# peterropac/Aegolius

Hardware: AMD Instinct MI355X
Metric: Mpoints/sec SDF eval, 1024^3 grid, 10-prim smooth-union tree (higher is better)
Workload: dtype f32

## Files before the change

### aegolius_amd/_engine.py

```python
import atexit
import contextlib
import ctypes
import importlib.util
import os
import sys
import threading

import numpy as np

_HERE = os.path.dirname(os.path.abspath(__file__))
LIB_PATH = os.path.join(_HERE, "libsdfk.so")

MODE_AUTO, MODE_INTERPRET, MODE_SPECIALIZED, MODE_NOCULL = 0, 1, 2, 3
(FLAVOUR_PLAIN_ARRAY, FLAVOUR_PLAIN_GRID, FLAVOUR_TILE_ARRAY, FLAVOUR_TILE_GRID, FLAVOUR_TILE_MASK, FLAVOUR_ROWS_ARRAY,
 FLAVOUR_ROWS_GRID, FLAVOUR_ROWS_MASK, FLAVOUR_ROWS2D_ARRAY, FLAVOUR_ROWS2D_GRID, FLAVOUR_RAYS, FLAVOUR_OCCUPANCY) = range(12)
FLAVOUR_FLAGS = 0x100
FLAVOUR_XY = 0x200

_c = ctypes
_vp, _i64, _int, _sz = _c.c_void_p, _c.c_int64, _c.c_int, _c.c_size_t
_fp = _c.POINTER(_c.c_float)

SIGNATURES = {
    "sdfk_abi_version": (_int, []),
    "sdfk_device_count": (_int, []),
    "sdfk_last_error": (_c.c_char_p, []),
    "sdfk_program_create": (_vp, [_vp, _sz, _vp, _sz, _vp, _sz, _int]),
    "sdfk_program_destroy": (None, [_vp]),
    "sdfk_program_set_params": (_int, [_vp, _vp, _sz]),
    "sdfk_program_set_cull": (_int, [_vp, _vp, _sz, _vp]),
    "sdfk_program_source": (_c.c_char_p, [_vp]),
    "sdfk_program_compile_check": (_int, [_vp, _c.POINTER(_sz)]),
    "sdfk_program_chain_members": (_int, [_vp]),
    "sdfk_program_compile_flavour": (_int, [_vp, _int, _c.POINTER(_sz), _c.POINTER(_c.c_double)]),
    "sdfk_debug_compile_external": (_int, [_vp, _int, _c.POINTER(_sz)]),
    "sdfk_debug_jit_stats": (None, [_c.POINTER(_i64), _c.POINTER(_c.c_double)]),
    "sdfk_jit_drain": (None, []),
    "sdfk_jit_cancel": (None, []),
    "sdfk_debug_set_rtc_defs": (None, [_c.c_char_p]),
    "sdfk_eval_device": (_int, [_vp, _vp, _i64, _i64, _vp, _vp, _int]),
    "sdfk_eval_device_rows": (_int, [_vp, _vp, _i64, _i64, _i64, _vp, _vp, _int]),
    "sdfk_eval_device_rows2d": (_int, [_vp, _vp, _i64, _i64, _i64, _vp, _vp, _int]),
    "sdfk_eval_device_rows2d_xy": (_int, [_vp, _vp, _i64, _i64, _i64, _vp, _vp, _int]),
    "sdfk_debug_cells_stats": (None, [_int, _c.POINTER(_c.c_longlong)]),
    "sdfk_debug_rays_stats": (None, [_int, _c.POINTER(_c.c_longlong)]),
    "sdfk_eval_device_rows3d": (_int, [_vp, _vp, _i64, _i64, _i64, _i64, _i64, _vp, _vp, _int]),
    "sdfk_debug_row_masks": (_int, [_vp, _vp, _i64, _i64, _i64, _vp, _c.POINTER(_i64), _c.POINTER(_int), _vp]),
    "sdfk_eval_grid_sharded": (_int, [_vp, _vp, _i64, _vp, _i64, _vp, _i64, _int, _vp, _vp, _int]),
    "sdfk_eval_grid_sharded_device": (_int, [_vp, _vp, _i64, _vp, _i64, _vp, _i64, _int, _vp, _int, _vp, _int]),
    "sdfk_eval_device_aux": (_int, [_vp, _vp, _i64, _i64, _vp, _int, _i64, _vp, _vp, _int]),
    "sdfk_eval_grid_aux": (_int, [_vp, _vp, _i64, _vp, _i64, _vp, _i64, _i64, _i64, _vp, _int, _i64, _vp, _vp, _int]),
    "sdfk_field_min": (_int, [_vp, _i64, _c.POINTER(_c.c_float), _vp]),
    "sdfk_grid_box_average": (_int, [_vp, _i64, _i64, _i64, _int, _int, _int, _int, _vp, _vp]),
    "sdfk_grid_edge_detect": (_int, [_vp, _i64, _i64, _i64, _vp, _vp]),
    "sdfk_debug_box_variant": (_int, [_i64, _i64, _i64, _int, _int, _int, _c.POINTER(_int)]),
    "sdfk_grid_signed": (_int, [_vp, _i64, _i64, _i64, _c.c_float, _int, _vp, _vp]),
    "sdfk_grid_boundary_mask": (_int, [_vp, _i64, _c.c_float, _vp, _vp]),
    "sdfk_grid_signed_slab": (_int, [_vp, _i64, _i64, _vp, _i64, _i64, _i64, _int, _vp, _vp]),
    "sdfk_eval_host": (_int, [_vp, _vp, _int, _i64, _i64, _vp, _int, _int]),
# ... 720 lines not shown
```

### aegolius_amd/csrc/sdfk.hip

```cpp
#include <hip/hip_runtime.h>
#include <hip/hiprtc.h>

#include <chrono>
#include <algorithm>
#include <atomic>
#include <cmath>
#include <condition_variable>
#include <cstdio>
#include <cstdlib>
#include <cstring>
#include <deque>
#include <functional>
#include <map>
#include <memory>
#include <mutex>
#include <thread>
#include <string>
#include <vector>
#include <dirent.h>
#include <dlfcn.h>
#include <fcntl.h>
#include <signal.h>
#include <spawn.h>
#include <sys/wait.h>
// ... 1045 lines not shown
    }
    e->cv.notify_all();
}
template <typename MakeSource>
static std::shared_ptr<CodeObject> code_get(const std::string& key, MakeSource make_source, int rwb, bool wait) {
    std::shared_ptr<CodeObject> e = code_entry(key);
    std::unique_lock<std::mutex> lk(e->mu);
    if (e->state == 3 && std::chrono::steady_clock::now() - e->failed_at > std::chrono::seconds(30)) e->state = 0;
    if (e->state == 0) {
        e->state = 1;
        lk.unlock();
        const std::string src = make_source();
        if (wait || !rtc_helper_available()) {
            code_build(e, src, rwb);
        } else {
            g_builds.post([e, src, rwb] { code_build(e, src, rwb, true); });
        }
        return e;
    }
    if (wait) e->cv.wait(lk, [&] { return e->state != 1; });
    return e;
}
static std::string flavour_key(const sdfk_program* p, int flavour, int rwb, int with_flags = 0) {
    return p->key + "|f" + std::to_string(flavour) + ((with_flags & 1) ? "s" : "") + ((with_flags & 2) ? "x" : "") + "|" + rtc_option_key(rwb);
}
static std::string flavour_source(const sdfk_program* p, int flavour, int with_flags = 0) {
    return std::string((with_flags & 1) ? "#define SDFK_FLAGS 1\n" : "") + ((with_flags & 2) ? "#define SDFK_XY 1\n" : "") +
           sdfk_generate_source(g_ops, SDFK_OP_COUNT, p->code.data(), p->code.size() / 2, p->result_reg, p->sites, flavour,
                                &p->sites_all);
}

extern "C" int sdfk_program_chain_members(const sdfk_program* p) {
    return p && p->chain_mode ? p->chain_members : 0;
}
extern "C" int sdfk_program_compile_check(sdfk_program* p, size_t* code_size) {
    if (!p) return fail(-1, "null program");
    size_t total = 0;
    const int rwb = rows_geo(p);
    for (int f = 0; f < SDFK_FL_COUNT; ++f) {
        if (f == SDFK_FL_RAYS) continue;
        if (f == SDFK_FL_OCCUPANCY) continue;
        if (p->sites.empty() && f != SDFK_FL_PLAIN_ARRAY && f != SDFK_FL_PLAIN_GRID) continue;
        if (p->chain_mode && (f == SDFK_FL_TILE_ARRAY || f == SDFK_FL_TILE_GRID || f == SDFK_FL_TILE_MASK || f == SDFK_FL_ROWS_MASK)) continue;
        std::shared_ptr<CodeObject> e = code_get(flavour_key(p, f, rwb), [&] { return flavour_source(p, f); }, rwb, true);
        if (e->state != 2) return fail(-3, e->error);
        total += e->co.size();
    }
    if (code_size) *code_size = total;
    return 0;
}
extern "C" int sdfk_program_compile_flavour(sdfk_program* p, int flavour, size_t* code_size, double* seconds) {
    if (!p) return fail(-1, "null program");
    int with_flags = 0;
    if (flavour >= 0 && (flavour & SDFK_FLAVOUR_FLAGS)) with_flags |= 1;
    if (flavour >= 0 && (flavour & SDFK_FLAVOUR_XY)) with_flags |= 2;
    if (flavour >= 0) flavour &= ~(SDFK_FLAVOUR_FLAGS | SDFK_FLAVOUR_XY);
    if (flavour < 0 || flavour >= SDFK_FL_COUNT) return fail(-1, "sdfk_program_compile_flavour: unknown flavour");
    if (p->sites.empty() && flavour != SDFK_FL_PLAIN_ARRAY && flavour != SDFK_FL_PLAIN_GRID && flavour != SDFK_FL_RAYS &&
        flavour != SDFK_FL_OCCUPANCY)
        return fail(-2, "sdfk_program_compile_flavour: the program has no cull sites");
    if (with_flags && flavour == SDFK_FL_RAYS)
        return fail(-2, "sdfk_program_compile_flavour: the ray flavour has no flag-writing or two-row build");
    if (with_flags && flavour == SDFK_FL_OCCUPANCY)
        return fail(-2, "sdfk_program_compile_flavour: the occupancy flavour has no flag-writing or two-row build");
    if ((with_flags & 2) && flavour != SDFK_FL_PLAIN_ARRAY && flavour != SDFK_FL_ROWS2D_ARRAY)
        return fail(-2, "sdfk_program_compile_flavour: two-row coordinates exist for the plain and the flat row-block array kernels");
    if ((with_flags & 1) && (flavour == SDFK_FL_TILE_ARRAY || flavour == SDFK_FL_TILE_GRID || flavour == SDFK_FL_TILE_MASK ||
                       flavour == SDFK_FL_ROWS_MASK))
        return fail(-2, "sdfk_program_compile_flavour: this flavour has no flag-writing build");
    const int rwb = rows_geo(p);
    const auto t0 = std::chrono::steady_clock::now();
    std::shared_ptr<CodeObject> e =
        code_get(flavour_key(p, flavour, rwb, with_flags), [&] { return flavour_source(p, flavour, with_flags); }, rwb, true);
    if (e->state != 2) return fail(-3, e->error);
    if (code_size) *code_size = e->co.size();
    if (seconds) *seconds = std::chrono::duration<double>(std::chrono::steady_clock::now() - t0).count();
    return 0;
}

extern "C" int sdfk_debug_compile_external(sdfk_program* p, int flavour, size_t* code_size) {
    if (!p) return fail(-1, "null program");
    if (flavour < 0 || flavour >= SDFK_FL_COUNT) return fail(-1, "sdfk_debug_compile_external: unknown flavour");
    if (p->sites.empty() && flavour != SDFK_FL_PLAIN_ARRAY && flavour != SDFK_FL_PLAIN_GRID && flavour != SDFK_FL_RAYS &&
        flavour != SDFK_FL_OCCUPANCY)
        return fail(-2, "sdfk_debug_compile_external: the program has no cull sites");
    if (!rtc_helper_available()) return fail(-9, "sdfk_rtc_helper is not next to libsdfk.so (or hiprtc cannot be located)");
    std::vector<char> co;
    std::string log;
    if (rtc_compile_external(flavour_source(p, flavour), &co, &log, rows_geo(p)) != 0) return fail(-3, log);
    if (code_size) *code_size = co.size();
    return 0;
}

static std::shared_ptr<SpecModule> get_module(sdfk_program* p, int device, int flavour, bool wait, std::string* err,
                                              int with_flags = 0) {
    const int rwb = rows_geo(p);
    const std::string key = flavour_key(p, flavour, rwb, with_flags);
    std::shared_ptr<SpecModule> m;
    {
        std::lock_guard<std::mutex> lk(g_code_mu);
        std::shared_ptr<SpecModule>& slot = g_mods[std::make_pair(device, key)];
        if (!slot) slot = std::make_shared<SpecModule>();
        m = slot;
    }
    std::lock_guard<std::mutex> lk(m->mu);
    if (m->loaded) return m;
    for (int attempt = 0;; ++attempt) {
        std::shared_ptr<CodeObject> e;
        {
            std::lock_guard<std::mutex> ce(g_code_mu);
            auto it = g_code.find(key);
            if (it != g_code.end()) e = it->second;
// ... 232 lines not shown
        for (const uint2& x : sp) {
            if (x.y == 0xffffffffu) ++all;
            else { sum += x.y; mx = std::max<unsigned long long>(mx, x.y); if (x.y == 0) ++empty; }
        }
        {
            std::lock_guard<std::mutex> lk(g_cells_stats_mu);
            g_cells_stats[0] = (long long)nf; g_cells_stats[1] = (long long)nc; g_cells_stats[2] = (long long)head;
            g_cells_stats[3] = (long long)cap; g_cells_stats[4] = (long long)sum; g_cells_stats[5] = (long long)mx;
            g_cells_stats[6] = (long long)all; g_cells_stats[7] = (long long)empty;
        }
        if (trace) fprintf(stderr, "[sdfk cells] %d members: fine %ux%ux%u = %llu cells (2^%u planes x 2^%u blocks x 2^%u windows), coarse %llu; pool %u of %llu entries; "
                "fine lists: mean %.1f max %llu, %llu without a list, %llu empty\n", p->chain_members, fine.ncx, fine.ncy, fine.ncz, nf, fine.lx, fine.ly, fine.lz, nc,
                head, cap, (double)sum / (double)std::max<unsigned long long>(1, nf - all - empty), mx, all, empty);
    }
    out->lv = fine;
    out->sph = b + o_fsph;
    out->span = b + o_fspan;
    out->cand = b + o_pool;
    out->enabled = 1u;
    out->ncells = (unsigned)nf;
    return 0;
}

static int run(sdfk_program* p, const SrcArray* arr, const SrcGrid* grid, long long n, float* d_out, void* stream_,
               int mode, bool vec_ok, long long row_len = 0, const float* aux = nullptr, long long aux_stride = 0,
               bool flat = false, long long plane_rows = 0, long long plane_phase = 0, unsigned* d_flags = nullptr,
               unsigned thr_key = 0, bool xy = false) {
    if (!p) return fail(-1, "null program");
    if (n < 0) return fail(-1, "negative point count");
    if (p->n_aux > 0 && (!aux || aux_stride < n))
        return fail(-1, "this program reads auxiliary fields (staged evaluation): use sdfk_eval_device_aux / sdfk_eval_grid_aux");
    if (n == 0) return 0;
    if (mode == SDFK_MODE_AUTO) mode = g_default_mode;
    if (d_flags && (mode == SDFK_MODE_AUTO || mode == SDFK_MODE_INTERPRET)) mode = SDFK_MODE_SPECIALIZED;
    if (xy) {
        if (!arr || p->n_aux > 0) return fail(-1, "two-row coordinates: array source, no auxiliary fields");
        if (mode == SDFK_MODE_AUTO || mode == SDFK_MODE_INTERPRET) mode = SDFK_MODE_SPECIALIZED;
    }
    hipStream_t stream = (hipStream_t)stream_;
    int device = 0;
    HIPCHK(hipGetDevice(&device));
    DevState* d = nullptr;
    int rc = ensure_resident(p, device, stream, &d);
    if (rc) return rc;

    long long n4 = vec_ok ? (n / 4) * 4 : 0;
    long long tail = n - n4;

    static const long long spec_limit = [] {
        const char* e = getenv("SDFK_SPECIALIZE_LIMIT");
// ... 12 lines not shown
    int flavour = arr ? SDFK_FL_PLAIN_ARRAY : SDFK_FL_PLAIN_GRID;
    const long long grow = grid ? (grid->n2 > 1 ? (long long)grid->n2 : (long long)grid->n1) : 0;
    if (!p->sites.empty() && mode != SDFK_MODE_NOCULL && mode != SDFK_MODE_INTERPRET) {
        if (arr && rows_geometry(n, row_len, &rg, (flat || d_flags) ? 0 : plane_rows, plane_phase, p->chain_mode))
            flavour = (flat || xy) ? SDFK_FL_ROWS2D_ARRAY : SDFK_FL_ROWS_ARRAY;
        else if (arr && vec_ok && !p->chain_mode && !d_flags && !xy) flavour = SDFK_FL_TILE_ARRAY;
        else if (grid && grid->start % grow == 0 &&
                 rows_geometry(n, grow, &rg, (grid->n2 > 1 && !d_flags) ? (long long)grid->n1 : 0,
                               grid->n2 > 1 ? (grid->start / grow) % (long long)grid->n1 : 0, p->chain_mode))
            flavour = grid->n2 > 1 ? SDFK_FL_ROWS_GRID : SDFK_FL_ROWS2D_GRID;
        else if (grid && vec_ok && !p->chain_mode && !d_flags) flavour = SDFK_FL_TILE_GRID;
        if (!p->chain_mode && (long long)(p->code.size() / 2) > rows_limit &&
            (flavour == SDFK_FL_ROWS_ARRAY || flavour == SDFK_FL_ROWS2D_ARRAY || flavour == SDFK_FL_ROWS_GRID || flavour == SDFK_FL_ROWS2D_GRID)) {
            const bool is_arr = arr != nullptr;
            if (vec_ok && !d_flags && !xy) flavour = is_arr ? SDFK_FL_TILE_ARRAY : SDFK_FL_TILE_GRID;
            else if (!d_flags) flavour = is_arr ? SDFK_FL_PLAIN_ARRAY : SDFK_FL_PLAIN_GRID;
        }
    }
    std::shared_ptr<SpecModule> sk;
    if (mode != SDFK_MODE_INTERPRET) {
        static const bool async_jit = [] { const char* e = getenv("SDFK_ASYNC_JIT"); return !(e && e[0] == '0'); }();
        const bool wait = mode != SDFK_MODE_AUTO || !p->interp_ok || !async_jit;
        std::string err;
        sk = get_module(p, device, flavour, wait, &err, (d_flags ? 1 : 0) | (xy ? 2 : 0));
        if (sk && sk->failed) {
            if (mode == SDFK_MODE_SPECIALIZED || !p->interp_ok)
                return fail(-3, "specialised kernel unavailable: " + err);
            static bool warned = false;
            if (!warned) {
                fprintf(stderr, "[sdfk] hiprtc specialisation failed, using the interpreter kernel: %s\n", err.c_str());
                warned = true;
            }
            sk.reset();
        }
    }
    if (!sk && !p->interp_ok)
        return fail(-4, "program needs more registers than the interpreter kernel has (use the specialised mode)");

    const float* prm = d->d_params;
    const float* tab = d->d_tables;
    if (sk) {
        if (flavour == SDFK_FL_ROWS_ARRAY || flavour == SDFK_FL_ROWS_GRID || flavour == SDFK_FL_ROWS2D_ARRAY ||
            flavour == SDFK_FL_ROWS2D_GRID) {
            const unsigned per_tile = (unsigned)(rows_waves(p) * rows_wbricks(p));
            const unsigned tiles = ((rg.nbricks + per_tile - 1) / per_tile + 127u) & ~127u;
            const unsigned rthreads = 64u * (unsigned)rows_waves(p);
            CellsArg cells{};
            const bool with_cells = p->chain_mode && sk->fn[1] != nullptr;
            if (arr) {
                const float* co = arr->co;
                long long stride = arr->stride;
                if (with_cells) {
                    void* src[] = {&co, &stride};
                    rc = prepare_cells(p, d, sk->fn[1], rg, src, 2, prm, tab, stream, &cells);
                    if (rc) return rc;
                }
                void* args[] = {&prm, &tab, &co, &stride, &rg, &d_out, &d_flags, &thr_key, &cells};
                HIPCHK(hipModuleLaunchKernel(sk->fn[0], tiles, 1, 1, rthreads, 1, 1, 0, stream, args, nullptr));
            } else {
                SrcGrid g = *grid;
                rg.row0 = grid->start / grow;
                rg.yrows = grid->n2 > 1 ? 0 : 1;
                if (with_cells) {
                    void* src[] = {&g};
                    rc = prepare_cells(p, d, sk->fn[1], rg, src, 1, prm, tab, stream, &cells);
                    if (rc) return rc;
                }
                void* args[] = {&prm, &tab, &g, &rg, &d_out, &d_flags, &thr_key, &cells};
                HIPCHK(hipModuleLaunchKernel(sk->fn[0], tiles, 1, 1, rthreads, 1, 1, 0, stream, args, nullptr));
            }
            return 0;
        }
        if (flavour == SDFK_FL_TILE_ARRAY || flavour == SDFK_FL_TILE_GRID) {
            const unsigned tiles = (unsigned)((n + tile_points() - 1) / tile_points());
            if (arr) {
                const float* co = arr->co;
                long long stride = arr->stride;
                void* args[] = {&prm, &tab, &co, &stride, &n, &d_out};
                HIPCHK(hipModuleLaunchKernel(sk->fn[0], tiles, 1, 1, tile_threads(), 1, 1, 0, stream, args, nullptr));
            } else {
                SrcGrid g = *grid;
                void* args[] = {&prm, &tab, &g, &n, &d_out};
                HIPCHK(hipModuleLaunchKernel(sk->fn[0], tiles, 1, 1, tile_threads(), 1, 1, 0, stream, args, nullptr));
            }
            return 0;
        }
        if (arr) {
            const float* co = arr->co;
            long long stride = arr->stride;
            if (n4) {
                long long off = 0;
// ... 196 lines not shown
    float* d = nullptr;
    ~AxisTables() {
        if (d) (void)hipFree(d);
    }
};

static int upload_axes(const float* ax0, int64_t n0, const float* ax1, int64_t n1, const float* ax2, int64_t n2,
                       hipStream_t stream, AxisTables* t, SrcGrid* g, int64_t start) {
    if (!ax0 || !ax1 || !ax2 || n0 < 1 || n1 < 1 || n2 < 1) return fail(-1, "grid axes missing or empty");
    if (n1 > 0x7fffffff || n2 > 0x7fffffff) return fail(-1, "grid axis too long");
    HIPCHK(hipMalloc(&t->d, (size_t)(n0 + n1 + n2) * sizeof(float)));
    HIPCHK(hipMemcpyAsync(t->d, ax0, (size_t)n0 * sizeof(float), hipMemcpyHostToDevice, stream));
    HIPCHK(hipMemcpyAsync(t->d + n0, ax1, (size_t)n1 * sizeof(float), hipMemcpyHostToDevice, stream));
    HIPCHK(hipMemcpyAsync(t->d + n0 + n1, ax2, (size_t)n2 * sizeof(float), hipMemcpyHostToDevice, stream));
    g->ax0 = t->d;
    g->ax1 = t->d + n0;
    g->ax2 = t->d + n0 + n1;
    g->n1 = (unsigned)n1;
    g->n2 = (unsigned)n2;
    g->start = start;
    return 0;
}

extern "C" int sdfk_eval_grid(sdfk_program* p, const float* ax0, int64_t n0, const float* ax1, int64_t n1,
                              const float* ax2, int64_t n2, int64_t start, int64_t count, float* d_out, void* stream,
                              int mode) {
    if (!d_out) return fail(-1, "sdfk_eval_grid: null output");
    if (start < 0 || count < 0 || start + count > n0 * n1 * n2) return fail(-1, "sdfk_eval_grid: range outside the grid");
    AxisTables t;
    SrcGrid g;
    int rc = upload_axes(ax0, n0, ax1, n1, ax2, n2, (hipStream_t)stream, &t, &g, start);
    if (rc) return rc;
    rc = run(p, nullptr, &g, count, d_out, stream, mode, aligned16(d_out));
    if (rc) return rc;
    HIPCHK(hipStreamSynchronize((hipStream_t)stream));
    return 0;
}

extern "C" int sdfk_eval_grid_aux(sdfk_program* p, const float* ax0, int64_t n0, const float* ax1, int64_t n1,
                                  const float* ax2, int64_t n2, int64_t start, int64_t count, const float* d_aux, int n_aux,
                                  int64_t aux_stride, float* d_out, void* stream, int mode) {
    if (!p || !d_out) return fail(-1, "sdfk_eval_grid_aux: null pointer");
    if (start < 0 || count < 0 || start + count > n0 * n1 * n2) return fail(-1, "sdfk_eval_grid_aux: range outside the grid");
    if (n_aux < p->n_aux) return fail(-1, "sdfk_eval_grid_aux: the program reads more auxiliary fields than were passed");
    AxisTables t;
    SrcGrid g;
    int rc = upload_axes(ax0, n0, ax1, n1, ax2, n2, (hipStream_t)stream, &t, &g, start);
    if (rc) return rc;
    rc = run(p, nullptr, &g, count, d_out, stream, mode, aligned16(d_out), 0, d_aux, aux_stride);
    if (rc) return rc;
    HIPCHK(hipStreamSynchronize((hipStream_t)stream));
    return 0;
}

extern "C" int sdfk_eval_grid_host(sdfk_program* p, const float* ax0, int64_t n0, const float* ax1, int64_t n1,
                                   const float* ax2, int64_t n2, int64_t start, int64_t count, float* out, int device,
                                   int mode) {
    if (!p) return fail(-1, "null program");
    if (count < 0 || (count > 0 && !out)) return fail(-1, "sdfk_eval_grid_host: bad arguments");
    if (start < 0 || start + count > n0 * n1 * n2) return fail(-1, "sdfk_eval_grid_host: range outside the grid");
    if (count == 0) return 0;
    HIPCHK(hipSetDevice(device));
    int64_t chunk = std::min<int64_t>(count, (int64_t)1 << 27);
    const int64_t grow = n2 > 1 ? n2 : n1;
    if (start % grow == 0 && chunk > grow) chunk = chunk / grow * grow;
    float* d_out = nullptr;
    HIPCHK(hipMalloc(&d_out, (size_t)chunk * sizeof(float)));
    AxisTables t;
    SrcGrid g;
    int rc = upload_axes(ax0, n0, ax1, n1, ax2, n2, nullptr, &t, &g, start);
    for (int64_t s = 0; s < count && rc == 0; s += chunk) {
        const int64_t m = std::min(chunk, count - s);
        g.start = start + s;
        rc = run(p, nullptr, &g, m, d_out, nullptr, mode, true);
        if (rc == 0 && hipMemcpy(out + s, d_out, (size_t)m * sizeof(float), hipMemcpyDeviceToHost) != hipSuccess)
            rc = fail(-6, "sdfk_eval_grid_host: device-to-host copy failed");
    }
    (void)hipFree(d_out);
    return rc;
}

extern "C" int sdfk_eval_grid_sharded(sdfk_program* p, const float* ax0, int64_t n0, const float* ax1, int64_t n1,
                                      const float* ax2, int64_t n2, int n_shards, const int* devices, float* out,
                                      int mode) {
    if (!p || !out) return fail(-1, "sdfk_eval_grid_sharded: null argument");
    if (n_shards < 1 || n_shards > 64) return fail(-1, "sdfk_eval_grid_sharded: 1..64 shards");
    if (!ax0 || !ax1 || !ax2 || n0 < 1 || n1 < 1 || n2 < 1) return fail(-1, "grid axes missing or empty");
    int n_dev = 0;
    if (hipGetDeviceCount(&n_dev) != hipSuccess || n_dev < 1) return fail(-8, "sdfk_eval_grid_sharded: no HIP device");
    const int64_t total = n0 * n1 * n2, unit = n2 > 1 ? n2 : n1;
    const int64_t per = (total / unit / n_shards) * unit;
    std::vector<int> rc((size_t)n_shards, 0);
    std::vector<std::string> msg((size_t)n_shards);
    std::vector<std::thread> workers;
    for (int d = 0; d < n_shards; ++d) {
        const int dev = devices ? devices[d] : d % n_dev;
        if (dev < 0 || dev >= n_dev) return fail(-1, "sdfk_eval_grid_sharded: device index out of range");
// ... 359 lines not shown
```

### aegolius_amd/csrc/sdfk_codegen.cpp

```cpp
#include "sdfk_codegen.h"

#include <algorithm>
#include <cstdio>
#include <cstring>
#include <map>
#include <set>

#include "sdfk_embedded.inc"

std::string sdfk_vector_prelude() { return std::string(kEmbeddedDevice) + "\n" + kEmbeddedVecdev + "\n"; }

static const char kWrappers[] = R"SDFKW(
template <int VEC, typename SRC>
static __device__ __forceinline__ void sdfk_body(const float* __restrict__ PRM, const float* __restrict__ TAB,
                                                 const SRC& src, long long off, long long n,
                                                 float* __restrict__ out, const float* __restrict__ aux,
                                                 long long aux_stride, unsigned* __restrict__ flags, unsigned thr) {
    const long long block_base = (long long)sdfk_bx() * (SDFK_BLOCK * VEC);
    const unsigned lane_off = sdfk_tx() * VEC;
#ifdef SDFK_FLAGS                                              // the flag-writing build of this flavour (its own code object:
    {                                                          // carried as a run-time branch it cost the field kernels registers)
        const bool active = block_base + lane_off < n;
        unsigned nib = 0u;
        if (active) {
// ... 1658 lines not shown
#else
#define SDFK_CELLS_KARG
#endif
)SDFKR";
static const char kRowsArray[] = R"SDFKR(
extern "C" __global__ __launch_bounds__(64 * SDFK_RWAVES) SDFK_ROWS_ATTR void sdfk_spec_r(
    const float* __restrict__ PRM, const float* __restrict__ TAB, const float* __restrict__ co, long long stride,
    sdfk_rowgeom g, float* __restrict__ out, unsigned* __restrict__ flags, unsigned thr SDFK_CELLS_KARG) {
    const SrcArray s = {co, stride};
    sdfk_rows_kernel(PRM, TAB, s, g, out, flags, thr SDFK_CELLS_PASS);
}
#ifdef SDFK_CELLS
extern "C" __global__ __launch_bounds__(256) void sdfk_spec_cells(
    const float* __restrict__ PRM, const float* __restrict__ TAB, const float* __restrict__ co, long long stride,
    sdfk_rowgeom g, sdfk_cellpass cp) {
    const SrcArray s = {co, stride};
    sdfk_cells_kernel(PRM, TAB, s, g, cp);
}
#endif
)SDFKR";
static const char kRowsGrid[] = R"SDFKR(
// the same on a regular grid expanded from three per-axis tables (no coordinate array: 4 B/point); the slab
// starts at a row boundary and out[0] is its first point
extern "C" __global__ __launch_bounds__(64 * SDFK_RWAVES) void sdfk_spec_rg(
    const float* __restrict__ PRM, const float* __restrict__ TAB, SrcGrid s, sdfk_rowgeom g, float* __restrict__ out,
    unsigned* __restrict__ flags, unsigned thr SDFK_CELLS_KARG) {
    sdfk_rows_kernel(PRM, TAB, s, g, out, flags, thr SDFK_CELLS_PASS);
}
#ifdef SDFK_CELLS
extern "C" __global__ __launch_bounds__(256) void sdfk_spec_cellsg(
    const float* __restrict__ PRM, const float* __restrict__ TAB, SrcGrid s, sdfk_rowgeom g, sdfk_cellpass cp) {
    sdfk_cells_kernel(PRM, TAB, s, g, cp);
}
#endif
)SDFKR";
static const char kRowsMask[] = R"SDFKR(
// test aid: the skip masks (two 64-bit words per brick: sites 0-31, 32-63; bit 2k = first operand of site k
// skipped, bit 2k+1 = second) followed by the "uniform rows" flag in a third word
extern "C" __global__ __launch_bounds__(64 * SDFK_RWAVES) void sdfk_spec_rmask(
    const float* __restrict__ PRM, const float* __restrict__ TAB, const float* __restrict__ co, long long stride,
    sdfk_rowgeom g, unsigned long long* __restrict__ masks) {
    __shared__ __attribute__((aligned(16))) sdfk_rowmeta meta;
    const SrcArray s = {co, stride};
    unsigned rb, c;
    sdfk_rows_prepare(PRM, TAB, s, g, &meta, sdfk_bx(), rb, c);
    const unsigned q = sdfk_bx() * SDFK_RNBRICK + sdfk_tx();
    if (sdfk_tx() < SDFK_RNBRICK && q < g.nbricks) {
        masks[3ull * q] = meta.mask[0][sdfk_tx()];
        masks[3ull * q + 1] = meta.mask[1][sdfk_tx()];
        masks[3ull * q + 2] = meta.uniform[sdfk_tx()];
    }
// ... 1000 lines not shown
```

### include/sdfk.h

```cpp
#ifndef SDFK_H
#define SDFK_H

#include <stddef.h>
#include <stdint.h>

#ifdef __cplusplus
extern "C" {
#endif

#define SDFK_ABI_VERSION 1

#define SDFK_MODE_AUTO 0
#define SDFK_MODE_INTERPRET 1
#define SDFK_MODE_SPECIALIZED 2
#define SDFK_MODE_NOCULL 3

typedef struct sdfk_program sdfk_program;

int sdfk_abi_version(void);
int sdfk_device_count(void);
const char* sdfk_last_error(void);

sdfk_program* sdfk_program_create(const uint32_t* code, size_t n_instr, const float* params, size_t n_params,
                                  const float* tables, size_t n_tables, int result_reg);
void sdfk_program_destroy(sdfk_program* prog);
int sdfk_program_set_params(sdfk_program* prog, const float* params, size_t n_params);
int sdfk_program_set_cull(sdfk_program* prog, const uint32_t* sites, size_t n_sites, const float* k);
int sdfk_program_chain_members(const sdfk_program* prog);
const char* sdfk_program_source(sdfk_program* prog);
int sdfk_program_compile_check(sdfk_program* prog, size_t* code_size);
#define SDFK_FLAVOUR_PLAIN_ARRAY 0
#define SDFK_FLAVOUR_PLAIN_GRID 1
#define SDFK_FLAVOUR_TILE_ARRAY 2
#define SDFK_FLAVOUR_TILE_GRID 3
#define SDFK_FLAVOUR_TILE_MASK 4
#define SDFK_FLAVOUR_ROWS_ARRAY 5
#define SDFK_FLAVOUR_ROWS_GRID 6
#define SDFK_FLAVOUR_ROWS_MASK 7
#define SDFK_FLAVOUR_ROWS2D_ARRAY 8
#define SDFK_FLAVOUR_ROWS2D_GRID 9
#define SDFK_FLAVOUR_RAYS 10
#define SDFK_FLAVOUR_OCCUPANCY 11
#define SDFK_FLAVOUR_FLAGS 0x100
#define SDFK_FLAVOUR_XY 0x200
int sdfk_program_compile_flavour(sdfk_program* prog, int flavour, size_t* code_size, double* seconds);
void sdfk_debug_cells_stats(int enable, long long* out8);
void sdfk_debug_rays_stats(int enable, long long* out8);
int sdfk_debug_compile_external(sdfk_program* prog, int flavour, size_t* code_size);
void sdfk_jit_drain(void);
void sdfk_jit_cancel(void);
void sdfk_debug_jit_stats(int64_t* builds, double* seconds);
void sdfk_debug_set_rtc_defs(const char* defs);

int sdfk_eval_device(sdfk_program* prog, const float* d_co, int64_t n, int64_t row_stride, float* d_out,
                     void* stream, int mode);
int sdfk_eval_device_rows(sdfk_program* prog, const float* d_co, int64_t n, int64_t row_stride, int64_t row_len,
                          float* d_out, void* stream, int mode);
int sdfk_eval_device_rows3d(sdfk_program* prog, const float* d_co, int64_t n, int64_t row_stride, int64_t row_len,
                            int64_t plane_rows, int64_t first_row_in_plane, float* d_out, void* stream, int mode);
int sdfk_eval_device_rows2d(sdfk_program* prog, const float* d_co, int64_t n, int64_t row_stride, int64_t row_len,
                            float* d_out, void* stream, int mode);
int sdfk_eval_device_rows2d_xy(sdfk_program* prog, const float* d_xy, int64_t n, int64_t row_stride, int64_t row_len,
                               float* d_out, void* stream, int mode);
int sdfk_eval_host(sdfk_program* prog, const void* co, int co_dtype, int64_t n, int64_t row_stride, float* out,
                   int device, int mode);
int sdfk_eval_host_resident(sdfk_program* prog, const void* co, int co_dtype, int64_t n, int64_t row_stride,
                            float* d_out, int device, int mode);
// ... 161 lines not shown
```

Baseline: 363,100.

## Add dedicated grid row-block kernel body for monotone axis tables with cached axes

Adds a specialised body for the grid row-block kernel, used when the host finds the axis tables monotone. It derives row indices on the scalar unit with a host-supplied reciprocal, computes probe spheres in closed form from table endpoints, and reads z straight from the axis table. This drops the coordinate staging and the uniformity vote and cuts LDS use, which should raise occupancy. The host also caches uploaded axis tables per device and builds a general variant for non-monotone tables, at the cost of an extra compiled variant and more code paths.

```diff
diff --git a/aegolius_amd/_engine.py b/aegolius_amd/_engine.py
--- a/aegolius_amd/_engine.py
+++ b/aegolius_amd/_engine.py
@@ -16,6 +16,7 @@
  FLAVOUR_ROWS_GRID, FLAVOUR_ROWS_MASK, FLAVOUR_ROWS2D_ARRAY, FLAVOUR_ROWS2D_GRID, FLAVOUR_RAYS, FLAVOUR_OCCUPANCY) = range(12)
 FLAVOUR_FLAGS = 0x100
 FLAVOUR_XY = 0x200
+FLAVOUR_GRID_GENERAL = 0x400
 
 _c = ctypes
 _vp, _i64, _int, _sz = _c.c_void_p, _c.c_int64, _c.c_int, _c.c_size_t
@@ -35,6 +36,7 @@
     "sdfk_program_compile_flavour": (_int, [_vp, _int, _c.POINTER(_sz), _c.POINTER(_c.c_double)]),
     "sdfk_debug_compile_external": (_int, [_vp, _int, _c.POINTER(_sz)]),
     "sdfk_debug_jit_stats": (None, [_c.POINTER(_i64), _c.POINTER(_c.c_double)]),
+    "sdfk_debug_last_grid_body": (_int, []),
     "sdfk_jit_drain": (None, []),
     "sdfk_jit_cancel": (None, []),
     "sdfk_debug_set_rtc_defs": (None, [_c.c_char_p]),
diff --git a/aegolius_amd/csrc/sdfk.hip b/aegolius_amd/csrc/sdfk.hip
--- a/aegolius_amd/csrc/sdfk.hip
+++ b/aegolius_amd/csrc/sdfk.hip
@@ -1091,10 +1091,12 @@
     return e;
 }
 static std::string flavour_key(const sdfk_program* p, int flavour, int rwb, int with_flags = 0) {
-    return p->key + "|f" + std::to_string(flavour) + ((with_flags & 1) ? "s" : "") + ((with_flags & 2) ? "x" : "") + "|" + rtc_option_key(rwb);
+    return p->key + "|f" + std::to_string(flavour) + ((with_flags & 1) ? "s" : "") + ((with_flags & 2) ? "x" : "") + ((with_flags & 4) ? "g" : "") + "|" +
+           rtc_option_key(rwb);
 }
 static std::string flavour_source(const sdfk_program* p, int flavour, int with_flags = 0) {
     return std::string((with_flags & 1) ? "#define SDFK_FLAGS 1\n" : "") + ((with_flags & 2) ? "#define SDFK_XY 1\n" : "") +
+           ((with_flags & 4) ? "#define SDFK_GRID_GENERAL 1\n" : "") +
            sdfk_generate_source(g_ops, SDFK_OP_COUNT, p->code.data(), p->code.size() / 2, p->result_reg, p->sites, flavour,
                                 &p->sites_all);
 }
@@ -1123,8 +1125,11 @@
     int with_flags = 0;
     if (flavour >= 0 && (flavour & SDFK_FLAVOUR_FLAGS)) with_flags |= 1;
     if (flavour >= 0 && (flavour & SDFK_FLAVOUR_XY)) with_flags |= 2;
-    if (flavour >= 0) flavour &= ~(SDFK_FLAVOUR_FLAGS | SDFK_FLAVOUR_XY);
+    if (flavour >= 0 && (flavour & SDFK_FLAVOUR_GRID_GENERAL)) with_flags |= 4;
+    if (flavour >= 0) flavour &= ~(SDFK_FLAVOUR_FLAGS | SDFK_FLAVOUR_XY | SDFK_FLAVOUR_GRID_GENERAL);
     if (flavour < 0 || flavour >= SDFK_FL_COUNT) return fail(-1, "sdfk_program_compile_flavour: unknown flavour");
+    if ((with_flags & 4) && flavour != SDFK_FL_ROWS_GRID)
+        return fail(-2, "sdfk_program_compile_flavour: only the grid row-block flavour has a build for general tables");
     if (p->sites.empty() && flavour != SDFK_FL_PLAIN_ARRAY && flavour != SDFK_FL_PLAIN_GRID && flavour != SDFK_FL_RAYS &&
         flavour != SDFK_FL_OCCUPANCY)
         return fail(-2, "sdfk_program_compile_flavour: the program has no cull sites");
@@ -1149,6 +1154,12 @@
 
 extern "C" int sdfk_debug_compile_external(sdfk_program* p, int flavour, size_t* code_size) {
     if (!p) return fail(-1, "null program");
+    int variant = 0;
+    if (flavour >= 0 && (flavour & SDFK_FLAVOUR_GRID_GENERAL)) {
+        flavour &= ~SDFK_FLAVOUR_GRID_GENERAL;
+        if (flavour != SDFK_FL_ROWS_GRID) return fail(-2, "sdfk_debug_compile_external: only the grid row-block flavour has a build for general tables");
+        variant = 4;
+    }
     if (flavour < 0 || flavour >= SDFK_FL_COUNT) return fail(-1, "sdfk_debug_compile_external: unknown flavour");
     if (p->sites.empty() && flavour != SDFK_FL_PLAIN_ARRAY && flavour != SDFK_FL_PLAIN_GRID && flavour != SDFK_FL_RAYS &&
         flavour != SDFK_FL_OCCUPANCY)
@@ -1156,7 +1167,7 @@
     if (!rtc_helper_available()) return fail(-9, "sdfk_rtc_helper is not next to libsdfk.so (or hiprtc cannot be located)");
     std::vector<char> co;
     std::string log;
-    if (rtc_compile_external(flavour_source(p, flavour), &co, &log, rows_geo(p)) != 0) return fail(-3, log);
+    if (rtc_compile_external(flavour_source(p, flavour, variant), &co, &log, rows_geo(p)) != 0) return fail(-3, log);
     if (code_size) *code_size = co.size();
     return 0;
 }
@@ -1435,10 +1446,13 @@
     return 0;
 }
 
+static thread_local int g_last_grid_body = -1;
+extern "C" int sdfk_debug_last_grid_body(void) { return g_last_grid_body; }
+
 static int run(sdfk_program* p, const SrcArray* arr, const SrcGrid* grid, long long n, float* d_out, void* stream_,
                int mode, bool vec_ok, long long row_len = 0, const float* aux = nullptr, long long aux_stride = 0,
                bool flat = false, long long plane_rows = 0, long long plane_phase = 0, unsigned* d_flags = nullptr,
-               unsigned thr_key = 0, bool xy = false) {
+               unsigned thr_key = 0, bool xy = false, bool grid_monotone = false) {
     if (!p) return fail(-1, "null program");
     if (n < 0) return fail(-1, "negative point count");
     if (p->n_aux > 0 && (!aux || aux_stride < n))
@@ -1497,7 +1511,13 @@
         static const bool async_jit = [] { const char* e = getenv("SDFK_ASYNC_JIT"); return !(e && e[0] == '0'); }();
         const bool wait = mode != SDFK_MODE_AUTO || !p->interp_ok || !async_jit;
         std::string err;
-        sk = get_module(p, device, flavour, wait, &err, (d_flags ? 1 : 0) | (xy ? 2 : 0));
+        int variant = (d_flags ? 1 : 0) | (xy ? 2 : 0);
+        if (flavour == SDFK_FL_ROWS_GRID && !d_flags && !p->chain_mode) {
+            const bool tables_body = grid_monotone && grid->start / grow + rg.R < 0x7fffffffLL && rg.L <= 0x40000000u;
+            if (!tables_body) variant |= 4;
+            g_last_grid_body = tables_body ? 1 : 0;
+        }
+        sk = get_module(p, device, flavour, wait, &err, variant);
         if (sk && sk->failed) {
             if (mode == SDFK_MODE_SPECIALIZED || !p->interp_ok)
                 return fail(-3, "specialised kernel unavailable: " + err);
@@ -1541,7 +1561,8 @@
                     rc = prepare_cells(p, d, sk->fn[1], rg, src, 1, prm, tab, stream, &cells);
                     if (rc) return rc;
                 }
-                void* args[] = {&prm, &tab, &g, &rg, &d_out, &d_flags, &thr_key, &cells};
+                unsigned inv_n1 = (unsigned)std::min<unsigned long long>(0xffffffffull, (1ull << 32) / (unsigned long long)g.n1);
+                void* args[] = {&prm, &tab, &g, &rg, &d_out, &d_flags, &thr_key, &inv_n1, &cells};
                 HIPCHK(hipModuleLaunchKernel(sk->fn[0], tiles, 1, 1, rthreads, 1, 1, 0, stream, args, nullptr));
             }
             return 0;
@@ -1784,16 +1805,86 @@
     return 0;
 }
 
+struct AxisEntry {
+    std::vector<float> host;
+    int64_t n0 = 0, n1 = 0, n2 = 0;
+    float* d = nullptr;
+    bool monotone = false;
+    ~AxisEntry() {
+        if (d) (void)hipFree(d);
+    }
+};
+static bool axis_monotone(const float* a, int64_t n) {
+    bool up = true, down = true;
+    for (int64_t i = 1; i < n; ++i) {
+        up = up && a[i] >= a[i - 1];
+        down = down && a[i] <= a[i - 1];
+    }
+    return up || down;
+}
+static constexpr size_t kAxisSlots = 4;
+struct AxisCache {
+    std::mutex mu;
+    std::map<int, std::vector<std::shared_ptr<AxisEntry>>> dev;
+};
+static AxisCache& axis_cache() {
+    static AxisCache* c = new AxisCache;
+    return *c;
+}
+static int cached_axes(const float* ax0, int64_t n0, const float* ax1, int64_t n1, const float* ax2, int64_t n2,
+                       std::shared_ptr<AxisEntry>* out, SrcGrid* g, int64_t start) {
+    if (!ax0 || !ax1 || !ax2 || n0 < 1 || n1 < 1 || n2 < 1) return fail(-1, "grid axes missing or empty");
+    if (n1 > 0x7fffffff || n2 > 0x7fffffff) return fail(-1, "grid axis too long");
+    int device = 0;
+    HIPCHK(hipGetDevice(&device));
+    std::shared_ptr<AxisEntry> e;
+    {
+        AxisCache& c = axis_cache();
+        std::lock_guard<std::mutex> lk(c.mu);
+        std::vector<std::shared_ptr<AxisEntry>>& slots = c.dev[device];
+        for (size_t i = 0; i < slots.size() && !e; ++i) {
+            const AxisEntry& s = *slots[i];
+            if (s.n0 == n0 && s.n1 == n1 && s.n2 == n2 && memcmp(s.host.data(), ax0, (size_t)n0 * sizeof(float)) == 0 &&
+                memcmp(s.host.data() + n0, ax1, (size_t)n1 * sizeof(float)) == 0 &&
+                memcmp(s.host.data() + n0 + n1, ax2, (size_t)n2 * sizeof(float)) == 0) {
+                e = slots[i];
+                std::rotate(slots.begin(), slots.begin() + (long)i, slots.begin() + (long)i + 1);
+            }
+        }
+        if (!e) {
+            e = std::make_shared<AxisEntry>();
+            e->n0 = n0; e->n1 = n1; e->n2 = n2;
+            e->host.resize((size_t)(n0 + n1 + n2));
+            memcpy(e->host.data(), ax0, (size_t)n0 * sizeof(float));
+            memcpy(e->host.data() + n0, ax1, (size_t)n1 * sizeof(float));
+            memcpy(e->host.data() + n0 + n1, ax2, (size_t)n2 * sizeof(float));
+            e->monotone = axis_monotone(ax0, n0) && axis_monotone(ax1, n1) && axis_monotone(ax2, n2);
+            HIPCHK(hipMalloc(&e->d, e->host.size() * sizeof(float)));
+            HIPCHK(hipMemcpy(e->d, e->host.data(), e->host.size() * sizeof(float), hipMemcpyHostToDevice));
+            if (slots.size() >= kAxisSlots) slots.pop_back();
+            slots.insert(slots.begin(), e);
+        }
+    }
+    g->ax0 = e->d;
+    g->ax1 = e->d + n0;
+    g->ax2 = e->d + n0 + n1;
+    g->n1 = (unsigned)n1;
+    g->n2 = (unsigned)n2;
+    g->start = start;
+    *out = e;
+    return 0;
+}
+
 extern "C" int sdfk_eval_grid(sdfk_program* p, const float* ax0, int64_t n0, const float* ax1, int64_t n1,
                               const float* ax2, int64_t n2, int64_t start, int64_t count, float* d_out, void* stream,
                               int mode) {
     if (!d_out) return fail(-1, "sdfk_eval_grid: null output");
     if (start < 0 || count < 0 || start + count > n0 * n1 * n2) return fail(-1, "sdfk_eval_grid: range outside the grid");
-    AxisTables t;
+    std::shared_ptr<AxisEntry> t;
     SrcGrid g;
-    int rc = upload_axes(ax0, n0, ax1, n1, ax2, n2, (hipStream_t)stream, &t, &g, start);
+    int rc = cached_axes(ax0, n0, ax1, n1, ax2, n2, &t, &g, start);
     if (rc) return rc;
-    rc = run(p, nullptr, &g, count, d_out, stream, mode, aligned16(d_out));
+    rc = run(p, nullptr, &g, count, d_out, stream, mode, aligned16(d_out), 0, nullptr, 0, false, 0, 0, nullptr, 0, false, t->monotone);
     if (rc) return rc;
     HIPCHK(hipStreamSynchronize((hipStream_t)stream));
     return 0;
@@ -1805,11 +1896,11 @@
     if (!p || !d_out) return fail(-1, "sdfk_eval_grid_aux: null pointer");
     if (start < 0 || count < 0 || start + count > n0 * n1 * n2) return fail(-1, "sdfk_eval_grid_aux: range outside the grid");
     if (n_aux < p->n_aux) return fail(-1, "sdfk_eval_grid_aux: the program reads more auxiliary fields than were passed");
-    AxisTables t;
+    std::shared_ptr<AxisEntry> t;
     SrcGrid g;
-    int rc = upload_axes(ax0, n0, ax1, n1, ax2, n2, (hipStream_t)stream, &t, &g, start);
+    int rc = cached_axes(ax0, n0, ax1, n1, ax2, n2, &t, &g, start);
     if (rc) return rc;
-    rc = run(p, nullptr, &g, count, d_out, stream, mode, aligned16(d_out), 0, d_aux, aux_stride);
+    rc = run(p, nullptr, &g, count, d_out, stream, mode, aligned16(d_out), 0, d_aux, aux_stride, false, 0, 0, nullptr, 0, false, t->monotone);
     if (rc) return rc;
     HIPCHK(hipStreamSynchronize((hipStream_t)stream));
     return 0;
@@ -1828,13 +1919,13 @@
     if (start % grow == 0 && chunk > grow) chunk = chunk / grow * grow;
     float* d_out = nullptr;
     HIPCHK(hipMalloc(&d_out, (size_t)chunk * sizeof(float)));
-    AxisTables t;
+    std::shared_ptr<AxisEntry> t;
     SrcGrid g;
-    int rc = upload_axes(ax0, n0, ax1, n1, ax2, n2, nullptr, &t, &g, start);
+    int rc = cached_axes(ax0, n0, ax1, n1, ax2, n2, &t, &g, start);
     for (int64_t s = 0; s < count && rc == 0; s += chunk) {
         const int64_t m = std::min(chunk, count - s);
         g.start = start + s;
-        rc = run(p, nullptr, &g, m, d_out, nullptr, mode, true);
+        rc = run(p, nullptr, &g, m, d_out, nullptr, mode, true, 0, nullptr, 0, false, 0, 0, nullptr, 0, false, t->monotone);
         if (rc == 0 && hipMemcpy(out + s, d_out, (size_t)m * sizeof(float), hipMemcpyDeviceToHost) != hipSuccess)
             rc = fail(-6, "sdfk_eval_grid_host: device-to-host copy failed");
     }
diff --git a/aegolius_amd/csrc/sdfk_codegen.cpp b/aegolius_amd/csrc/sdfk_codegen.cpp
--- a/aegolius_amd/csrc/sdfk_codegen.cpp
+++ b/aegolius_amd/csrc/sdfk_codegen.cpp
@@ -1704,11 +1704,281 @@
 static const char kRowsGrid[] = R"SDFKR(
 // the same on a regular grid expanded from three per-axis tables (no coordinate array: 4 B/point); the slab
 // starts at a row boundary and out[0] is its first point
+//
+// Field-writing builds of 3-D grids whose axis tables are monotone (the host checks them when it uploads them and
+// otherwise builds the SDFK_GRID_GENERAL variant) get a body of their own around the same generated per-point code.
+// Same bricks, same enumeration, same workgroup, same probe and fold; what is gone is everything the array body does to
+// find out what axis tables state outright:
+//   row -> (ix, iy)   once per brick on the scalar unit, with floor(2^32 / n1) from the host (inv_n1; the host takes this
+//                     body only while the slab's global rows stay below 2^31); a lane adds its row and wraps
+//   probe spheres     closed form: the box spanned by the table entries at a sub-brick's first / last row and first / last
+//                     column bounds every point of it (monotone tables); nothing is staged to be re-read
+//   phase-C z         the lane's 8 values straight from ax2 (a few KB, cache resident), issued before the probe
+//   no z / xy staging, no uniformity vote (rows have one x and one y by construction): 3.7 KB of LDS instead of 21 KB for
+//   the 10-leaf tree
+// -DSDFK_GRIDBODY=0 restores the array body (A/B: tools/rows_ab.py grid:base grid:GRIDBODY=0).
+#ifndef SDFK_GRIDBODY
+#define SDFK_GRIDBODY 1
+#endif
+#if SDFK_GRIDBODY && !defined(SDFK_GRID_GENERAL) && defined(SDFK_SIMT) && !defined(SDFK_CHAIN) && !defined(SDFK_CELLS) && \
+    !defined(SDFK_FLAT) && !defined(SDFK_FLAGS)
+struct sdfk_gridmeta {
+    unsigned long long mask[SDFK_NMASK][SDFK_RNBRICK];
+    float4 cen[SDFK_NCEN];
+    float leafval[SDFK_NLEAF * SDFK_NCEN];
+};
+#define SDFK_GNZP (SDFK_NSUB >= 4 ? 4 : 1)       // sub-bricks along the window ...
+#define SDFK_GNRP (SDFK_NSUB / SDFK_GNZP)        // ... and across the rows (sdfk_sub_centre's shapes; one sub-brick: the brick)
+#define SDFK_GRPS (SDFK_RROWS / SDFK_GNRP)
+#define SDFK_GZPS (SDFK_RZ / SDFK_GNZP)
+static_assert(SDFK_GZPS % (2 * SDFK_NP) == 0, "a lane's points lie in one sub-brick");
+// row dr of a block whose first row is (ix0, iy0)
+static __device__ __forceinline__ void sdfk_grid_row(unsigned ix0, unsigned iy0, unsigned dr, unsigned n1, unsigned& ix, unsigned& iy) {
+    ix = ix0;
+    iy = iy0 + dr;
+    while (iy >= n1) { iy -= n1; ++ix; }
+}
+// rows of sub-brick row group `gr` of a block of nrows live rows: halves / quarters of the 16 rows — but two groups split
+// where iy wraps (the block's rows come from two planes), so that each part lies in one plane (sdfk_sub_centre's rule)
+static __device__ __forceinline__ unsigned sdfk_grid_split(unsigned iy0, unsigned nrows, unsigned n1) {
+    const unsigned s1 = n1 - iy0;                // rows before iy wraps (>= 1)
+    return (SDFK_GNRP == 2 && s1 < nrows) ? s1 : SDFK_GRPS;
+}
+static __device__ __forceinline__ unsigned sdfk_grid_group(unsigned row, unsigned split) {
+    return SDFK_GNRP == 2 ? (row >= split ? 1u : 0u) : row / SDFK_GRPS;
+}
+// Probe sphere of sub-brick sb of window k of the block [r0, r0 + nrows) (local rows; first row = (ix0, iy0)): midpoint and
+// half-diagonal of the box of the table entries at its extreme indices. Window k of local row r starts (r * L) mod 32
+// points before column 32 k, a shift that wraps from row to row: the column range is the union over the rows, clamped to
+// the row in edge windows. Rows past the end of the block count as its last row (they are evaluated as copies of it).
+static __device__ __forceinline__ float4 sdfk_grid_centre(const SrcGrid& s, unsigned L, long long r0, unsigned nrows, unsigned ix0,
+                                                          unsigned iy0, unsigned k, unsigned sb) {
+#ifdef SDFK_ABLATE_BOUNDS
+    return make_float4(0.0f, 0.0f, 0.0f, 1.0f);
+#else
+    const unsigned gr = sb / SDFK_GNZP, split = sdfk_grid_split(iy0, nrows, s.n1);
+    unsigned ra = gr * SDFK_GRPS, rb = ra + SDFK_GRPS - 1u;                 // rows [ra, rb] of the block
+    if (SDFK_GNRP == 2) { ra = gr ? split : 0u; rb = gr ? SDFK_RROWS - 1u : split - 1u; }
+    ra = min(ra, nrows - 1u);
+    rb = min(rb, nrows - 1u);
+    unsigned ixa, iya, ixb, iyb;
+    sdfk_grid_row(ix0, iy0, ra, s.n1, ixa, iya);
+    sdfk_grid_row(ix0, iy0, rb, s.n1, ixb, iyb);
+    if (ixa != ixb) { iya = 0u; iyb = s.n1 - 1u; }                          // several planes: every y of the axis
+    const unsigned sh0 = ((unsigned)r0 * L) & 31u, dl = L & 31u;
+    unsigned smin = 31u, smax = 0u;
+    for (unsigned r = ra; r <= rb; ++r) {
+        const unsigned sh = (sh0 + r * dl) & 31u;
+        smin = min(smin, sh);
+        smax = max(smax, sh);
+    }
+    const int i0 = (int)(32u * k + (sb % SDFK_GNZP) * SDFK_GZPS), last = (int)L - 1;
+    const int za = min(max(i0 - (int)smax, 0), last), ze = min(max(i0 + SDFK_GZPS - 1 - (int)smin, 0), last);
+    const float xa = s.ax0[ixa], xb = s.ax0[ixb], ya = s.ax1[iya], yb = s.ax1[iyb], z0 = s.ax2[za], z1 = s.ax2[ze];
+    const float cx = 0.5f * (xa + xb), cy = 0.5f * (ya + yb), cz = 0.5f * (z0 + z1);
+    const float dx = sd_rawmax(sd_abs(xa - cx), sd_abs(xb - cx)), dy = sd_rawmax(sd_abs(ya - cy), sd_abs(yb - cy));
+    const float dz = sd_rawmax(sd_abs(z0 - cz), sd_abs(z1 - cz));
+    const float r2 = sd_fma(dz, dz, sd_fma(dx, dx, dy * dy));
+    return make_float4(cx, cy, cz, 1.00001f * sqrtf(r2) + 1e-30f);
+#endif
+}
+struct sdfk_gridlane {                           // what a lane needs of one brick in phase C
+    float x, y;
+    float4 za, zb;                               // its 8 z values
+    long long f;                                 // flat index of its first point
+    int z;                                       // ... and its index in the row (edge windows: may lie outside)
+    bool live_row;
+};
+static __device__ __forceinline__ float4 sdfk_grid_z4(const float* __restrict__ ax2, int z, int last, bool interior) {
+    if (interior) {
+        const sdfk_f4u v = *reinterpret_cast<const sdfk_f4u*>(ax2 + z);
+        return make_float4(v.x, v.y, v.z, v.w);
+    }
+    return make_float4(ax2[min(max(z, 0), last)], ax2[min(max(z + 1, 0), last)], ax2[min(max(z + 2, 0), last)],
+                       ax2[min(max(z + 3, 0), last)]);
+}
+// the lane's part of window k of the block [r0, r0 + nrows) whose first row is (ix0, iy0)
+static __device__ __forceinline__ sdfk_gridlane sdfk_grid_lane(const SrcGrid& s, unsigned L, long long r0, unsigned nrows, unsigned ix0,
+                                                               unsigned iy0, unsigned k, unsigned lr, int zq) {
+    sdfk_gridlane me;
+    const bool interior = sdfk_interior(L, k);
+    me.live_row = lr < nrows;
+    const unsigned dr = me.live_row ? lr : nrows - 1u;
+    unsigned ix, iy;
+    sdfk_grid_row(ix0, iy0, dr, s.n1, ix, iy);
+    me.x = s.ax0[ix];
+    me.y = s.ax1[iy];
+    me.z = sdfk_win_z(r0 + dr, L, k, zq, &me.f);
+    me.za = sdfk_grid_z4(s.ax2, me.z, (int)L - 1, interior);
+    me.zb = sdfk_grid_z4(s.ax2, me.z + 4, (int)L - 1, interior);
+    return me;
+}
+#ifndef SDFK_GRID_HOIST
+#define SDFK_GRID_HOIST 0
+#endif                                           // against 2.03 — occupancy hides that latency better than registers do
+static __device__ __forceinline__ void sdfk_grid_kernel(const float* __restrict__ PRM, const float* __restrict__ TAB,
+                                                        const SrcGrid& s, const sdfk_rowgeom& g, unsigned inv_n1,
+                                                        float* __restrict__ out) {
+    __shared__ __attribute__((aligned(16))) sdfk_gridmeta meta;
+    const int lane = sdfk_tx() & 63, wave = __builtin_amdgcn_readfirstlane(sdfk_tx() >> 6);
+    const unsigned lr = (unsigned)lane / SDFK_RLPR;
+    const int zq = (lane % SDFK_RLPR) * (2 * SDFK_NP);
+    const int last = (int)g.L - 1;
+#ifndef SDFK_RTILES
+#define SDFK_RTILES 1
+#endif
+#ifndef SDFK_XGROUP
+#define SDFK_XGROUP (SDFK_RNBRICK <= 4 ? 16 : (SDFK_RNBRICK <= 8 ? 8 : 4))    // (sdfk_rows_kernel: the same tile mapping)
+#endif
+#pragma unroll 1
+  for (unsigned tt = 0; tt < SDFK_RTILES; ++tt) {
+    const unsigned xg_t = sdfk_bx() / 8;
+    const unsigned tile = (((xg_t / SDFK_XGROUP) * 8 + sdfk_bx() % 8) * SDFK_XGROUP + xg_t % SDFK_XGROUP) * SDFK_RTILES + tt;
+    if (tile * SDFK_RNBRICK >= g.nbricks) break;
+    if (tt) __syncthreads();
+    const unsigned q0 = tile * SDFK_RNBRICK + wave * SDFK_RWBRICKS;            // first brick of this wave
+    unsigned rb = sdfk_udiv(q0, g.nchunk, g.inv_nchunk);
+    unsigned c = q0 - rb * g.nchunk;
+    // the wave's bricks: scalars and the probe spheres (SDFK_GRID_HOIST: the lanes' coordinates too)
+    long long br0[SDFK_RWBRICKS];
+    unsigned bnrows[SDFK_RWBRICKS], bix0[SDFK_RWBRICKS], biy0[SDFK_RWBRICKS], bk[SDFK_RWBRICKS];
+#if SDFK_GRID_HOIST
+    sdfk_gridlane gl[SDFK_RWBRICKS];
+#endif
+    float4 cc = make_float4(0.0f, 0.0f, 0.0f, 1.0f);                           // (a dead brick still meets a fold lane: harmless values)
+#pragma unroll
+    for (int j = 0; j < SDFK_RWBRICKS; ++j) {
+        long long r0, rend;
+        sdfk_block_rows(g, rb, r0, rend);
+        const bool live = q0 + j < g.nbricks && r0 < rend;
+        br0[j] = r0;
+        bk[j] = c;
+        bnrows[j] = live ? (unsigned)(rend - r0 < SDFK_RROWS ? rend - r0 : SDFK_RROWS) : 0u;
+        const unsigned g0 = live ? (unsigned)(g.row0 + r0) : 0u;
+        bix0[j] = sdfk_udiv(g0, s.n1, inv_n1);
+        biy0[j] = g0 - bix0[j] * s.n1;
+        if (++c == g.nchunk) { c = 0; ++rb; }
+        if (!live) continue;
+#if SDFK_GRID_HOIST
+        gl[j] = sdfk_grid_lane(s, g.L, r0, bnrows[j], bix0[j], biy0[j], bk[j], lr, zq);
+#endif
+        if ((unsigned)lane / SDFK_NSUB == (unsigned)j && lane < SDFK_RWBRICKS * SDFK_NSUB)
+            cc = sdfk_grid_centre(s, g.L, r0, bnrows[j], bix0[j], biy0[j], bk[j], (unsigned)lane % SDFK_NSUB);
+    }
+    if (lane < SDFK_RWBRICKS * SDFK_NSUB) meta.cen[wave * (SDFK_RWBRICKS * SDFK_NSUB) + lane] = cc;
+    if (lane < SDFK_RWBRICKS) {
+#pragma unroll
+        for (int w = 0; w < SDFK_NMASK; ++w)
+#ifdef SDFK_ABLATE_PROBE
+            meta.mask[w][wave * SDFK_RWBRICKS + lane] = 0ull;
+#else
+            meta.mask[w][wave * SDFK_RWBRICKS + lane] = ~0ull;                  // the fold lanes AND their decisions into these
+#endif
+    }
+    __syncthreads();
+#ifndef SDFK_ABLATE_PROBE
+    sdfk_probe_leaves(meta.cen, meta.leafval, PRM, TAB);
+    __syncthreads();
+    if (sdfk_tx() < SDFK_NCEN && tile * SDFK_RNBRICK + sdfk_tx() / SDFK_NSUB < g.nbricks) {
+        const float4 pc = meta.cen[sdfk_tx()];
+        V3T<float> ctr = {pc.x, pc.y, pc.z};
+        unsigned long long mk[SDFK_NMASK];
+        sdfk_probe_fold(meta.leafval, sdfk_tx(), ctr, pc.w, PRM, mk);
+#pragma unroll
+        for (int w = 0; w < SDFK_NMASK; ++w)
+            __hip_atomic_fetch_and(&meta.mask[w][sdfk_tx() / SDFK_NSUB], mk[w], __ATOMIC_RELAXED, __HIP_MEMORY_SCOPE_WORKGROUP);
+    }
+    __syncthreads();
+#endif
+#pragma unroll 1
+    for (int j = 0; j < SDFK_RWBRICKS; ++j) {
+        if (q0 + j >= g.nbricks) break;
+        const int b = wave * SDFK_RWBRICKS + j;
+        // (the loop stays rolled — the generated code is emitted once — so the brick's values are SELECTED, not indexed)
+        unsigned nrows = bnrows[0], k = bk[0], ix0 = bix0[0], iy0 = biy0[0];
+        long long r0 = br0[0];
+#pragma unroll
+        for (int t = 1; t < SDFK_RWBRICKS; ++t)
+            if (j == t) { nrows = bnrows[t]; k = bk[t]; ix0 = bix0[t]; iy0 = biy0[t]; r0 = br0[t]; }
+        if (nrows == 0u) continue;
+#if SDFK_GRID_HOIST
+        sdfk_gridlane me = gl[0];
+#pragma unroll
+        for (int t = 1; t < SDFK_RWBRICKS; ++t)
+            if (j == t) me = gl[t];
+#else
+        const sdfk_gridlane me = sdfk_grid_lane(s, g.L, r0, nrows, ix0, iy0, k, lr, zq);
+#endif
+        unsigned mw[2 * SDFK_NMASK];                             // the brick's skip bits as scalar words
+#pragma unroll
+        for (int w = 0; w < SDFK_NMASK; ++w) {
+            const unsigned long long m = meta.mask[w][b];
+            mw[2 * w] = __builtin_amdgcn_readfirstlane((unsigned)m);
+            mw[2 * w + 1] = __builtin_amdgcn_readfirstlane((unsigned)(m >> 32));
+        }
+        const bool interior = sdfk_interior(g.L, k);
+#ifdef SDFK_ABLATE_EDGE
+        if (!interior) continue;
+#endif
+        V3P P[SDFK_NP];
+        f2 res[SDFK_NP];
+        P[0].z = {me.za.x, me.za.y};
+        P[1].z = {me.za.z, me.za.w};
+        P[2].z = {me.zb.x, me.zb.y};
+        P[3].z = {me.zb.z, me.zb.w};
+#ifdef SDFK_ABLATE_EVAL
+        SDFK_EACH res[q] = P[q].z + __builtin_bit_cast(float, mw[0] ^ mw[1] ^ mw[2] ^ mw[3]);
+#else
+        SDFK_EACH { P[q].x = sp<f2>(me.x); P[q].y = sp<f2>(me.y); }
+        sdfk_rows_culled<true>(me.x, me.y, P, mw, PRM, TAB, res);
+#endif
+#ifdef SDFK_DEBUG_BOUND
+        {   // test aid: instead of the field, component SDFK_DEBUG_BOUND (cx, cy, cz, rho) of the probe sphere of the
+            // sub-brick that holds the point
+            const unsigned row = me.live_row ? lr : nrows - 1u;
+            const unsigned sb = sdfk_grid_group(row, sdfk_grid_split(iy0, nrows, s.n1)) * SDFK_GNZP + (unsigned)zq / SDFK_GZPS;
+            const float4 dc = meta.cen[b * SDFK_NSUB + sb];
+            const float dv = SDFK_DEBUG_BOUND == 0 ? dc.x : (SDFK_DEBUG_BOUND == 1 ? dc.y : (SDFK_DEBUG_BOUND == 2 ? dc.z : dc.w));
+            SDFK_EACH res[q] = sp<f2>(dv);
+        }
+#endif
+        if (me.live_row) {
+            float* po = out + me.f;
+            if (interior) {
+#pragma unroll
+                for (int q = 0; q < SDFK_NP; q += 2) {
+                    sdfk_f4u v = {res[q].x, res[q].y, res[q + 1].x, res[q + 1].y};
+#ifdef SDFK_GRID_PLAINSTORE
+                    *reinterpret_cast<sdfk_f4u*>(po + 2 * q) = v;
+#else
+                    __builtin_nontemporal_store(v, reinterpret_cast<sdfk_f4u*>(po + 2 * q));
+#endif
+                }
+            } else {
+                SDFK_EACH {
+                    if (me.z + 2 * q >= 0 && me.z + 2 * q <= last) po[2 * q] = res[q].x;
+                    if (me.z + 2 * q + 1 >= 0 && me.z + 2 * q + 1 <= last) po[2 * q + 1] = res[q].y;
+                }
+            }
+        }
+    }
+  }
+}
+extern "C" __global__ __launch_bounds__(64 * SDFK_RWAVES) SDFK_ROWS_ATTR void sdfk_spec_rg(
+    const float* __restrict__ PRM, const float* __restrict__ TAB, SrcGrid s, sdfk_rowgeom g, float* __restrict__ out,
+    unsigned* __restrict__ flags, unsigned thr, unsigned inv_n1) {
+    (void)flags;
+    (void)thr;
+    sdfk_grid_kernel(PRM, TAB, s, g, inv_n1, out);
+}
+#else
 extern "C" __global__ __launch_bounds__(64 * SDFK_RWAVES) void sdfk_spec_rg(
     const float* __restrict__ PRM, const float* __restrict__ TAB, SrcGrid s, sdfk_rowgeom g, float* __restrict__ out,
-    unsigned* __restrict__ flags, unsigned thr SDFK_CELLS_KARG) {
+    unsigned* __restrict__ flags, unsigned thr, unsigned inv_n1 SDFK_CELLS_KARG) {
+    (void)inv_n1;
     sdfk_rows_kernel(PRM, TAB, s, g, out, flags, thr SDFK_CELLS_PASS);
 }
+#endif
 #ifdef SDFK_CELLS
 extern "C" __global__ __launch_bounds__(256) void sdfk_spec_cellsg(
     const float* __restrict__ PRM, const float* __restrict__ TAB, SrcGrid s, sdfk_rowgeom g, sdfk_cellpass cp) {
diff --git a/include/sdfk.h b/include/sdfk.h
--- a/include/sdfk.h
+++ b/include/sdfk.h
@@ -43,6 +43,8 @@
 #define SDFK_FLAVOUR_OCCUPANCY 11
 #define SDFK_FLAVOUR_FLAGS 0x100
 #define SDFK_FLAVOUR_XY 0x200
+#define SDFK_FLAVOUR_GRID_GENERAL 0x400
+int sdfk_debug_last_grid_body(void);
 int sdfk_program_compile_flavour(sdfk_program* prog, int flavour, size_t* code_size, double* seconds);
 void sdfk_debug_cells_stats(int enable, long long* out8);
 void sdfk_debug_rays_stats(int enable, long long* out8);
```

Result: no change. 363,500, median of 6 (+0.1%).
